# HandSomeWay/myGauHuman

Hardware: AMD Instinct MI355X
Metric: frames/sec fwd+bwd @1024^2, 200k Gaussians (higher is better)
Workload: dtype f32

## Files before the change

### mygauhuman_amd/csrc/geometry.hip

```cpp
#include "expand.h"
#include "gsr_common.h"
#include "project.h"
#include "sh_math.h"

namespace gsr {

constexpr int SH_M = 16;
constexpr int SH_ROW = SH_M * 3;
constexpr int SH_HALF = SH_ROW / 2;
constexpr int SH_LDS_ROW = 28;
constexpr int SH_CPT = SH_HALF / 4;

template <bool STAGE_SH>
__global__ __launch_bounds__(PRE_BLOCK) void preprocess_forward_kernel(const PreprocessArgs a) {
  __shared__ uint32_t wave_tot[PRE_BLOCK / WAVE];
  __shared__ __attribute__((aligned(16))) float s_sh[STAGE_SH ? PRE_BLOCK * SH_LDS_ROW : 4];
  const int i = blockIdx.x * PRE_BLOCK + threadIdx.x;
  float4 second[STAGE_SH ? SH_CPT : 1];
  if (STAGE_SH) {
    const int first = blockIdx.x * PRE_BLOCK;
    const int nrows = min(PRE_BLOCK, a.P - first);
    if (a.sh_half) {
      const uint4 *slab = reinterpret_cast<const uint4 *>(reinterpret_cast<const _Float16 *>(a.shs) + (size_t)first * SH_ROW);
#pragma unroll
// ... 67 lines not shown
            want_sh = true;
          } else {
            rgb = sh_to_rgb(a.D, p, a.campos, a.shs + (size_t)i * a.M * 3, clamp_bits);
          }
          my_radius = radi;
          tiles = area;
          rec.x = pix;
          rec.y = piy;
          rec.conic_a = cv.z * det_inv;
          rec.conic_b = -cv.y * det_inv;
          rec.conic_c = cv.x * det_inv;
          rec.opacity = a.opacities[i];
          rec.depth = pv.z;
          rec.r = rgb.x;
          rec.g = rgb.y;
          rec.b = rgb.z;
          const float o = rec.opacity, t255 = 255.0f * o;
          float hx = __builtin_inff(), hy = __builtin_inff();
          if (o == o) {
            if (!(t255 >= 1.0f)) {
              hx = hy = -1.0e30f;
            } else if (cv.x > 0.f && cv.z > 0.f && det > 0.f) {
              const float tau2 = 2.0f * (logf(t255) + 0.02f);
              hx = sqrtf(tau2 * cv.x) * 1.0001f + 0.01f;
              hy = sqrtf(tau2 * cv.z) * 1.0001f + 0.01f;
            }
          }
          rec.hx = hx;
          rec.hy = hy;
        }
      }
    }
  }
  if (STAGE_SH) {
    float3 d0;
    const ShDir dir = sh_dir(p, a.campos, d0);
    float res[3] = {0.f, 0.f, 0.f};
    __syncthreads();
    if (want_sh) sh_accumulate<0, SH_M / 2>(a.D, dir, &s_sh[threadIdx.x * SH_LDS_ROW], res);
    __syncthreads();
    {
      const int nrows = min(PRE_BLOCK, a.P - blockIdx.x * PRE_BLOCK);
      if (a.sh_half) {
#pragma unroll
        for (int j = 0; j < SH_CPT / 2; j++) {
          const int e = (int)threadIdx.x + j * PRE_BLOCK, row = e / (SH_CPT / 2), c8 = e % (SH_CPT / 2);
          if (row < nrows) {
            const _Float16 *hv = reinterpret_cast<const _Float16 *>(&second[j]);
            float *dst = &s_sh[row * SH_LDS_ROW + 8 * c8];
#pragma unroll
            for (int e2 = 0; e2 < 8; e2++) dst[e2] = (float)hv[e2];
          }
        }
      } else {
#pragma unroll
        for (int j = 0; j < SH_CPT; j++) {
          const int e = (int)threadIdx.x + j * PRE_BLOCK, row = e / SH_CPT, c4 = e % SH_CPT;
          if (row < nrows) *reinterpret_cast<float4 *>(&s_sh[row * SH_LDS_ROW + 4 * c4]) = second[j];
        }
      }
    }
    __syncthreads();
    if (want_sh) {
      sh_accumulate<SH_M / 2, SH_M>(a.D, dir, &s_sh[threadIdx.x * SH_LDS_ROW], res);
      const float3 rgb = sh_finish(res, clamp_bits);
      rec.r = rgb.x;
      rec.g = rgb.y;
      rec.b = rgb.z;
    }
  }
  if (i < a.P) {
    a.radii[i] = my_radius;
    a.geom.tiles_touched[i] = tiles;
    a.geom.clamped[i] = (uint8_t)clamp_bits;
    float4 *dst = reinterpret_cast<float4 *>(a.geom.recs + i);
    dst[0] = make_float4(rec.x, rec.y, rec.conic_a, rec.conic_b);
    dst[1] = make_float4(rec.conic_c, rec.opacity, rec.depth, rec.r);
    dst[2] = make_float4(rec.g, rec.b, rec.hx, rec.hy);
    if (a.zero_rows) {
      float4 *row = reinterpret_cast<float4 *>(a.geom.grad_rows + (size_t)i * GROWX);
#pragma unroll
      for (int k = 0; k < GROWX / 4; k++) row[k] = make_float4(0.f, 0.f, 0.f, 0.f);
    }
  }
  const uint32_t incl_w = wave_incl_scan(tiles);
  const int wave = threadIdx.x / WAVE, lane = threadIdx.x % WAVE;
  if (lane == WAVE - 1) wave_tot[wave] = incl_w;
  __syncthreads();
  uint32_t base = 0;
#pragma unroll
  for (int w = 0; w < PRE_BLOCK / WAVE; w++)
    if (w < wave) base += wave_tot[w];
  const uint32_t incl = base + incl_w;
  if (i < a.P) a.geom.block_incl[i] = incl;
  if (threadIdx.x == PRE_BLOCK - 1) a.geom.block_sums[blockIdx.x] = incl;
}

int launch_preprocess_forward(const PreprocessArgs &a, hipStream_t stream) {
  if (a.P <= 0) return GSR_OK;
  const bool stage = a.shs && !a.colors_precomp && a.M == SH_M && (reinterpret_cast<size_t>(a.shs) % 16 == 0);
  if (a.sh_half && a.shs && !a.colors_precomp && !stage) {
    set_error("fp16 SH storage needs 16 coefficients per Gaussian and a 16-byte aligned array");
    return GSR_EINVAL;
  }
  if (stage)
    hipLaunchKernelGGL(preprocess_forward_kernel<true>, dim3(pre_blocks(a.P)), dim3(PRE_BLOCK), 0, stream, a);
  else
    hipLaunchKernelGGL(preprocess_forward_kernel<false>, dim3(pre_blocks(a.P)), dim3(PRE_BLOCK), 0, stream, a);
  return GSR_OK;
}

__global__ void mark_visible_kernel(int P, const float *means3D, const float *view, uint8_t *present) {
  const int i = blockIdx.x * blockDim.x + threadIdx.x;
  if (i >= P) return;
  const float3 p = make_float3(means3D[3 * i], means3D[3 * i + 1], means3D[3 * i + 2]);
  const float z = view[2] * p.x + view[6] * p.y + view[10] * p.z + view[14];
// ... 104 lines not shown
```

### mygauhuman_amd/csrc/gsr_api.hip

```cpp
#include <stdarg.h>
#include <stdio.h>
#include <string.h>

#include <atomic>
#include <mutex>
#include <string>
#include <unordered_map>
#include <utility>
#include <vector>

#include "gsr_common.h"

namespace gsr {

static thread_local std::string g_error;

void set_error(const char *fmt, ...) {
  char buf[1024];
  va_list ap;
  va_start(ap, fmt);
  vsnprintf(buf, sizeof(buf), fmt, ap);
  va_end(ap);
  g_error = buf;
}
// ... 88 lines not shown
  } else if (!strcmp(key, "bucket_sort_merged")) {
    if (v != 0 && v != 1) return bad("0 or 1");
    o.bucket_sort_merged = v;
  } else if (!strcmp(key, "blend_sort")) {
    if (v != 0 && v != 1) return bad("0 or 1");
    o.blend_sort = v;
  } else if (!strcmp(key, "tile_order")) {
    if (v < 0 || v > 3) return bad("0 (natural order), 1 (longest lists first), 2 / 3 (2 x 2 / 4 x 2 tile blocks by summed length, a block per XCD)");
    o.tile_order = v;
  } else if (!strcmp(key, "tile_cull")) {
    if (v != 0 && v != 1) return bad("0 or 1");
    o.tile_cull = v;
  } else if (!strcmp(key, "blend_bwd_reduce")) {
    if (v < 0 || v > 4) return bad("0 (permlane / DPP folds), 3 (LDS folds: default); experiments: 1 (MFMA on folded rows), 2 (transposed MFMA contraction), 4 (LDS folds, the round-3 kernel)");
    if (experiment(v == 1 || v == 2 || v == 4)) return GSR_EINVAL;
    o.blend_bwd_reduce = v;
  } else if (!strcmp(key, "blend_layout")) {
    if (v != 0 && v != 1) return bad("0 (quadrant waves) or 1 (experiment: 4x4 blocks, four survivors per step)");
    if (experiment(v == 1)) return GSR_EINVAL;
    o.blend_layout = v;
  } else if (!strcmp(key, "blend_tail_cut")) {
    if (v < 0 || v > 16) return bad("0 .. 16 (sixteenths of the busy tiles at the end of the visiting order)");
    o.blend_tail_cut = v;
  } else if (!strcmp(key, "blend_segments")) {
    if (v < 0 || v > 64) return bad("0 (never) or the outlier threshold in quarters of the frame's mean list length (4 .. 64)");
    o.blend_segments = v;
  } else if (!strcmp(key, "blend_prio")) {
    if (v < 0 || v > 4) return bad("0, 1 (issue priority by list length); experiments: 2..4 (MEASUREMENT ONLY: render the longest lists alone)");
    if (experiment(v >= 2)) return GSR_EINVAL;
    o.blend_prio = v;
  } else if (!strcmp(key, "bake_batch_cells")) {
    if (v < 0 || v > 1000) return bad("0 (as many as the workspace holds) or 1 .. 1000");
    o.bake_batch_cells = v;
  } else if (!strcmp(key, "debug_no_atomics")) {
    if (v != 0 && v != 1) return bad("0 or 1");
    o.debug_no_atomics = v;
  } else if (!strcmp(key, "deterministic")) {
    if (v != 0 && v != 1) return bad("0 or 1");
    o.deterministic = v;
  } else {
    set_error("unknown tuning key %s", key);
    return GSR_EINVAL;
  }
  return GSR_OK;
}

static int readback_u32x2(const uint32_t *dev, uint32_t *out, hipStream_t stream) {
  ApiState &st = S();
  uint32_t *pinned = nullptr;
  {
    std::lock_guard<std::mutex> lock(st.pin_mutex);
    if (!st.pin_free.empty()) {
      pinned = st.pin_free.back();
      st.pin_free.pop_back();
    }
  }
  if (!pinned) GSR_HIP(hipHostMalloc(reinterpret_cast<void **>(&pinned), 64, hipHostMallocDefault));
  hipError_t e = hipMemcpyAsync(pinned, dev, 2 * sizeof(uint32_t), hipMemcpyDeviceToHost, stream);
  if (e == hipSuccess) e = hipStreamSynchronize(stream);
  out[0] = pinned[0];
  out[1] = pinned[1];
  {
    std::lock_guard<std::mutex> lock(st.pin_mutex);
    st.pin_free.push_back(pinned);
  }
  GSR_HIP(e);
// ... 200 lines not shown
}

int forward_stage_a(const FwdIn &in, const GeomState &geom, int *radii, hipStream_t stream, bool skip_scan = false) {
  const int grid_x = (in.width + TILE - 1) / TILE, grid_y = (in.height + TILE - 1) / TILE;
  PreprocessArgs pa;
  memset(&pa, 0, sizeof(pa));
  pa.P = in.P;
  pa.D = in.D;
  pa.M = in.M;
  pa.means3D = in.means3D;
  pa.scales = in.scales;
  pa.rotations = in.rotations;
  pa.opacities = in.opacities;
  pa.shs = in.shs;
  pa.cov3D_precomp = in.cov3D_precomp;
  pa.colors_precomp = in.colors_precomp;
  pa.scale_modifier = in.scale_modifier;
  pa.view = in.viewmatrix;
  pa.proj = in.projmatrix;
  pa.campos = in.cam_pos;
  pa.W = in.width;
  pa.H = in.height;
  pa.grid_x = grid_x;
  pa.grid_y = grid_y;
  pa.tan_fovx = in.tan_fovx;
  pa.tan_fovy = in.tan_fovy;
  pa.focal_y = in.height / (2.0f * in.tan_fovy);
  pa.focal_x = in.width / (2.0f * in.tan_fovx);
  pa.radii = radii;
  pa.geom = geom;
  pa.prefiltered = in.prefiltered;
  pa.sh_half = in.sh_half;
  pa.zero_rows = (in.debug & GSR_FWD_ZERO_ROWS) ? 1 : 0;
  if (in.prefiltered) GSR_HIP(zero_async(geom.total + 1, sizeof(uint32_t), stream));
  prof_begin(PROF_PREPROCESS_FWD, stream);
  int rc = launch_preprocess_forward(pa, stream);
  prof_end(PROF_PREPROCESS_FWD, stream);
  if (rc != GSR_OK) return rc;
  GSR_LAUNCH_CHECK(stream, in.debug & 1);
  if (skip_scan) return GSR_OK;
  prof_begin(PROF_SCAN, stream);
  rc = launch_scan_block_sums(geom, in.P, stream);
  prof_end(PROF_SCAN, stream);
  if (rc != GSR_OK) return rc;
  GSR_LAUNCH_CHECK(stream, in.debug & 1);
  return GSR_OK;
}

int forward_stage_b(const FwdIn &in, const GeomState &geom, BinningState &bin, const ImageState &img, const int *radii,
                    long R_host, size_t capacity, uint32_t *dev_status, hipStream_t stream, bool scan_fused = false) {
  const Options opt = options_for(stream);
  const int grid_x = (in.width + TILE - 1) / TILE, grid_y = (in.height + TILE - 1) / TILE;
  const size_t tiles = (size_t)grid_x * grid_y;
  int rc;
  const bool bucket = R_host < 0 || opt.binning_mode == GSR_BINNING_TILE_BUCKET;
  const bool fwd_sorts = bucket && forward_sorts_lists(opt, in.n_extra) && bucket_uses_hist(opt, in.P, tiles, capacity);
  prof_begin(PROF_BINNING, stream);
  if (bucket) {
    const int segments = (opt.tile_order == 1 && opt.blend_layout == 0 && !opt.blend_fwd_dma && (in.n_extra != 0 || opt.blend_fwd_waves == 4))
                             ? (opt.blend_segments | (opt.blend_tail_cut << 8)) : 0;
    rc = bucket_binning(geom, radii, in.P, grid_x, grid_y, capacity, R_host < 0, bin, img.ranges, img.order, img.ckpt_base, segments,
                        dev_status, in.prefiltered != 0, scan_fused, fwd_sorts, opt, stream, in.debug & 1);
    if (rc != GSR_OK) return rc;
  } else {
    const size_t R = (size_t)R_host;
    const int end_bit = 32 + (int)higher_msb((uint32_t)tiles);
// ... 327 lines not shown
  pb.means3D = means3D;
  pb.shs = shs;
  pb.scales = scales;
  pb.rotations = rotations;
  pb.cov3D = cov3D_precomp ? cov3D_precomp : geom.cov3D;
  pb.radii = radii;
  pb.clamped = geom.clamped;
  pb.scale_modifier = scale_modifier;
  pb.view = viewmatrix;
  pb.proj = projmatrix;
  pb.campos = campos;
  pb.W = width;
  pb.H = height;
  pb.tan_fovx = tan_fovx;
  pb.tan_fovy = tan_fovy;
  pb.focal_y = height / (2.0f * tan_fovy);
  pb.focal_x = width / (2.0f * tan_fovx);
  pb.grad_rows = geom.grad_rows;
  pb.grow = grow;
  pb.clear_rows = (flags & GSR_BWD_ROWS_ZEROED) ? 1 : 0;
  pb.CE = n_extra;
  pb.sh_half = sh_dtype == GSR_SH_F16 ? 1 : 0;
  pb.dL_dextra = dL_dextra;
  pb.recs = geom.recs;
  pb.dL_dmean2D = dL_dmean2D;
  pb.dL_dconic = dL_dconic;
  pb.dL_dopacity = dL_dopacity;
  pb.dL_dcolor = dL_dcolor;
  pb.dL_dmean3D = dL_dmean3D;
  pb.dL_dcov3D = dL_dcov3D;
  pb.dL_dsh = dL_dsh;
  pb.dL_dscale = dL_dscale;
  pb.dL_drot = dL_drot;
  prof_begin(PROF_PREPROCESS_BWD, stream);
  rc = launch_preprocess_backward(pb, stream);
  prof_end(PROF_PREPROCESS_BWD, stream);
  if (det_rows) {
    (void)hipStreamSynchronize(stream);
    (void)hipFree(det_rows);
  }
  if (rc != GSR_OK) return rc;
  GSR_LAUNCH_CHECK(stream, debug);
  return GSR_OK;
}

int gsr_rasterize_backward_ex(int P, int D, int M, int R, const float *background, int width, int height, const float *means3D,
                              const float *shs, const float *colors_precomp, const float *alphas, const float *scales,
                              float scale_modifier, const float *rotations, const float *cov3D_precomp, const float *viewmatrix,
                              const float *projmatrix, const float *campos, float tan_fovx, float tan_fovy, const int *radii,
                              char *geom_buffer, char *binning_buffer, char *image_buffer, const float *dL_dpix,
                              const float *dL_ddepths, const float *dL_dalphas, float *dL_dmean2D, float *dL_dconic,
                              float *dL_dopacity, float *dL_dcolor, float *dL_dmean3D, float *dL_dcov3D, float *dL_dsh,
                              float *dL_dscale, float *dL_drot, int debug, const float *extra_features, int n_extra,
                              const float *const *dL_dout_extra, float *dL_dextra, int sh_dtype, gsr_stream_t stream) {
  return rasterize_backward_impl(nullptr, nullptr, P, D, M, R, background, width, height, means3D, shs, colors_precomp, alphas, scales,
                                 scale_modifier, rotations, cov3D_precomp, viewmatrix, projmatrix, campos, tan_fovx, tan_fovy, radii,
                                 geom_buffer, binning_buffer, image_buffer, dL_dpix, dL_ddepths, dL_dalphas, dL_dmean2D, dL_dconic,
                                 dL_dopacity, dL_dcolor, dL_dmean3D, dL_dcov3D, dL_dsh, dL_dscale, dL_drot, debug, extra_features,
                                 n_extra, dL_dout_extra, dL_dextra, sh_dtype, stream);
}

int gsr_rasterize_backward_colors(int P, int R, int width, int height, char *geom_buffer, char *binning_buffer, char *image_buffer,
                                  const float *dL_dpix, float *dL_dcolor, int n_extra, const float *const *dL_dout_extra,
                                  float *dL_dextra, int debug, gsr_stream_t stream_) {
  hipStream_t stream = reinterpret_cast<hipStream_t>(stream_);
  if (P < 0 || R < 0 || width <= 0 || height <= 0) {
// ... 213 lines not shown
```

### mygauhuman_amd/csrc/gsr_common.h

```cpp
#pragma once
#include <hip/hip_runtime.h>
#include <stdint.h>
#include <stddef.h>

#include "../../include/gsr.h"

namespace gsr {

constexpr int TILE = 16;
constexpr int WAVE = 64;
constexpr int PRE_BLOCK = 256;

struct alignas(16) SplatRec {
  float x, y, conic_a, conic_b;
  float conic_c, opacity, depth, r;
  float g, b, hx, hy;
};
static_assert(sizeof(SplatRec) == 48, "SplatRec layout");

constexpr int GROW = 16;

constexpr int GROWX = 32;
constexpr int CE_MAX = 18;

struct GeomState {
  SplatRec *recs;
  float *cov3D;
  uint8_t *clamped;
  uint32_t *tiles_touched;
  uint32_t *point_offsets;
  int *internal_radii;
  uint32_t *block_incl;
  uint32_t *block_sums;
  uint32_t *block_prefix;
  uint32_t *total;
  float *grad_rows;
};
struct BinningState {
  uint64_t *keys_a;
  uint32_t *vals_a;
  uint64_t *keys_s;
  uint32_t *vals_s;
  uint32_t *hist;
  uint32_t *tile_counts;
  uint32_t *tile_cursor;
};
struct ImageState {
  float *final_T;
  uint32_t *n_contrib;
  uint2 *ranges;
  uint32_t *order;
  uint32_t *ckpt_base;
  float *ckpt;
};

inline size_t align_up(size_t v, size_t a) { return (v + a - 1) / a * a; }
template <typename T>
inline void carve(uintptr_t &p, T *&out, size_t count) {
  p = align_up(p, 256);
  out = reinterpret_cast<T *>(p);
  p += count * sizeof(T);
}
inline uintptr_t carve_begin(const void *chunk) { return reinterpret_cast<uintptr_t>(chunk); }

inline int pre_blocks(int P) { return (P + PRE_BLOCK - 1) / PRE_BLOCK; }
constexpr int SORT_ITEMS = 16;
constexpr int SORT_BLOCK = 256;
constexpr int SORT_TILE = SORT_ITEMS * SORT_BLOCK;
inline size_t sort_blocks(size_t n) { return (n + SORT_TILE - 1) / SORT_TILE; }
inline size_t sort_hist_words(size_t n) { return 256 * (sort_blocks(n) ? sort_blocks(n) : 1) + 256; }

inline GeomState geom_from_chunk(char *chunk_, size_t P, size_t *end = nullptr) {
  GeomState g;
  uintptr_t chunk = carve_begin(chunk_);
  size_t nb = (size_t)pre_blocks((int)P);
  carve(chunk, g.recs, P);
  carve(chunk, g.cov3D, P * 6);
  carve(chunk, g.clamped, P);
  carve(chunk, g.tiles_touched, P);
  carve(chunk, g.point_offsets, P);
  carve(chunk, g.internal_radii, P);
  carve(chunk, g.block_incl, P);
  carve(chunk, g.block_sums, nb);
  carve(chunk, g.block_prefix, nb);
  carve(chunk, g.total, 4);
  carve(chunk, g.grad_rows, P * GROWX);
  if (end) *end = chunk;
  return g;
}
inline size_t geom_bytes(size_t P) {
  size_t end = 0;
  geom_from_chunk(nullptr, P, &end);
  return end + 256;
}
inline BinningState binning_from_chunk(char *chunk_, size_t R, size_t tiles = 0, size_t *end = nullptr) {
  BinningState b;
  uintptr_t chunk = carve_begin(chunk_);
  size_t n = R ? R : 1;
  carve(chunk, b.keys_a, n);
  carve(chunk, b.vals_a, n);
  carve(chunk, b.keys_s, n);
  carve(chunk, b.vals_s, n);
  carve(chunk, b.hist, sort_hist_words(n));
  b.tile_counts = b.tile_cursor = nullptr;
  if (tiles) {
    carve(chunk, b.tile_counts, tiles * 16);
    carve(chunk, b.tile_cursor, tiles);
  }
  if (end) *end = chunk;
  return b;
}
inline size_t binning_bytes(size_t R, size_t tiles) {
  size_t end = 0;
  binning_from_chunk(nullptr, R, tiles ? tiles : 1, &end);
  return end + 256;
}
#if defined(__HIPCC__)
#define GSR_HD __host__ __device__
#else
// ... 52 lines not shown
  do {                                                                       \
    int _rc = ::gsr::check_hip((expr), #expr, __FILE__, __LINE__);           \
    if (_rc != GSR_OK) return _rc;                                           \
  } while (0)
#define GSR_LAUNCH_CHECK(stream, debug)                                      \
  do {                                                                       \
    GSR_HIP(hipGetLastError());                                              \
    if (debug) GSR_HIP(hipStreamSynchronize(stream));                        \
  } while (0)

enum ProfStage { PROF_PREPROCESS_FWD = 0, PROF_SCAN = 1, PROF_BINNING = 2, PROF_BLEND_FWD = 3, PROF_BLEND_BWD = 4,
                 PROF_PREPROCESS_BWD = 5, PROF_BLEND_BWD_COLORS = 6, PROF_NSTAGES = 7 };
void prof_begin(int stage, hipStream_t stream);
void prof_end(int stage, hipStream_t stream);

struct Options {
  int binning_mode = GSR_BINNING_TILE_BUCKET;
  int tile_cull = 1;
  int tile_order = 1;
  int bucket_hist = 1;
  int bucket_sort_merged = 1;
  int blend_sort = 1;
  int bucket_cstride = 4;
  int blend_fwd_dma = 0;
  int blend_fwd_waves = 4;
  int blend_bwd_waves = 4;
  int blend_bwd_reduce = 3;
  int deterministic = 0;
  int blend_layout = 0;
  int blend_tail_cut = 0;
  int blend_segments = 8;
  int blend_prio = 1;
  int bake_batch_cells = 0;
  int debug_no_atomics = 0;
};
Options options_for(hipStream_t stream);

struct PreprocessArgs {
  int P, D, M;
  const float *means3D, *scales, *rotations, *opacities, *shs, *cov3D_precomp, *colors_precomp;
  float scale_modifier;
  const float *view, *proj, *campos;
  int W, H, grid_x, grid_y;
  float tan_fovx, tan_fovy, focal_x, focal_y;
  int *radii;
  GeomState geom;
  int prefiltered;
  int sh_half;
  int zero_rows;
};
int launch_preprocess_forward(const PreprocessArgs &a, hipStream_t stream);
int launch_mark_visible(int P, const float *means3D, const float *view, uint8_t *present, hipStream_t stream);
int launch_scan_block_sums(const GeomState &g, int P, hipStream_t stream);
int launch_duplicate(const GeomState &g, const int *radii, int P, int grid_x, int grid_y, uint64_t *keys,
                     uint32_t *vals, hipStream_t stream);
int radix_sort_u64(size_t n, const uint64_t *in_k, const uint32_t *in_v, uint64_t *x_k, uint32_t *x_v, uint64_t *y_k,
                   uint32_t *y_v, int end_bit, uint32_t *hist, hipStream_t stream, int debug);
int radix_sort_u32(size_t n, const uint32_t *in_k, const uint32_t *in_v, uint32_t *x_k, uint32_t *x_v, uint32_t *y_k,
                   uint32_t *y_v, int end_bit, uint32_t *hist, hipStream_t stream, int debug);
inline int radix_passes(int end_bit) { return (end_bit + 7) / 8; }
int launch_tile_ranges(size_t R, const uint64_t *keys_sorted, uint2 *ranges, size_t tiles, hipStream_t stream);

struct BlendFwdArgs {
  const uint32_t *order;
  const uint2 *ranges;
  uint32_t *point_list;
  const SplatRec *recs;
  const uint64_t *unsorted;
  uint64_t *keys_sorted;
  int W, H, grid_x, grid_y;
  const float *bg;
  float *out_color, *out_depth, *out_alpha, *final_T;
  uint32_t *n_contrib;
  const float *extra;
  int CE;
  float *out_extra;
  int list_prio;
  const uint32_t *ckpt_base;
  float *ckpt;
  unsigned long long *trace;
};
int launch_blend_forward(const BlendFwdArgs &a, const Options &opt, hipStream_t stream);
// ... 59 lines not shown
struct BlendColorsBwdArgs {
  const uint32_t *order;
  const uint2 *ranges;
  const uint32_t *point_list;
  const SplatRec *recs;
  int W, H, grid_x, grid_y;
  const float *g_img[CB_IMAGES];
  int n_img;
  uint64_t col0;
  uint32_t col_mask;
  float *dL_dextra;
  float *dL_dcolor;
  int list_prio;
};
int launch_blend_colors_backward(const BlendColorsBwdArgs &a, hipStream_t stream);

struct PreprocessBwdArgs {
  int P, D, M;
  const float *means3D, *shs, *scales, *rotations, *cov3D;
  const int *radii;
  const uint8_t *clamped;
  float scale_modifier;
  const float *view, *proj, *campos;
  int W, H;
  float tan_fovx, tan_fovy, focal_x, focal_y;
  float *grad_rows;
  int grow;
  int clear_rows;
  int CE;
  float *dL_dextra;
  const SplatRec *recs;
  float *dL_dmean2D, *dL_dconic, *dL_dopacity, *dL_dcolor, *dL_dmean3D, *dL_dcov3D, *dL_dsh, *dL_dscale, *dL_drot;
  int sh_half;
};
int launch_preprocess_backward(const PreprocessBwdArgs &a, hipStream_t stream);

int launch_query_recs(int what, int P, const GeomState &g, void *dst, hipStream_t stream);

int bucket_binning(const GeomState &g, const int *radii, int P, int grid_x, int grid_y, size_t capacity, bool device_sized,
                   BinningState &b, uint2 *ranges, uint32_t *order, uint32_t *ckpt_base, int segments, uint32_t *dev_status,
                   bool check_prefilter, bool scan_fused, bool fwd_sorts, const Options &opt, hipStream_t stream, int debug);
bool bucket_uses_hist(const Options &opt, int P, size_t tiles, size_t capacity);
int bucket_sort_lists(const uint2 *ranges, uint64_t *bucket, uint32_t *point_list, uint64_t *keys_sorted, uint32_t *big_list,
                      uint32_t *big_count, size_t tiles, hipStream_t stream);

}

#if defined(__HIPCC__)
namespace gsr {

__device__ __forceinline__ int f2i_sat(float f) {
  if (f != f) return 0;
  if (f >= 2147483648.0f) return 2147483647;
  if (f <= -2147483648.0f) return (-2147483647 - 1);
  return (int)f;
}

__device__ __forceinline__ void tile_rect(float px, float py, int radius, int gx, int gy, int &x0, int &y0, int &x1,
                                          int &y1) {
  const float r = (float)radius;
  x0 = min(gx, max(0, f2i_sat((px - r) / (float)TILE)));
  y0 = min(gy, max(0, f2i_sat((py - r) / (float)TILE)));
  x1 = min(gx, max(0, f2i_sat((px + r + (float)(TILE - 1)) / (float)TILE)));
  y1 = min(gy, max(0, f2i_sat((py + r + (float)(TILE - 1)) / (float)TILE)));
}

// ... 74 lines not shown
```

### mygauhuman_amd/csrc/preprocess_bwd.hip

```cpp
#include "gsr_common.h"
#include "sh_math.h"

namespace gsr {

__device__ __forceinline__ void cov3d_backward(const float3 sc, float mod, const float4 q, const float *d, float *dL_dscale,
                                               float *dL_drot) {
  const float r = q.x, x = q.y, y = q.z, z = q.w;
  float R[3][3];
  R[0][0] = 1.f - 2.f * (y * y + z * z);
  R[0][1] = 2.f * (x * y - r * z);
  R[0][2] = 2.f * (x * z + r * y);
  R[1][0] = 2.f * (x * y + r * z);
  R[1][1] = 1.f - 2.f * (x * x + z * z);
  R[1][2] = 2.f * (y * z - r * x);
  R[2][0] = 2.f * (x * z - r * y);
  R[2][1] = 2.f * (y * z + r * x);
  R[2][2] = 1.f - 2.f * (x * x + y * y);
  const float s[3] = {mod * sc.x, mod * sc.y, mod * sc.z};
  float M[3][3];
#pragma unroll
  for (int c = 0; c < 3; c++)
#pragma unroll
    for (int rr = 0; rr < 3; rr++) M[c][rr] = s[rr] * R[c][rr];
  const float dS[3][3] = {{d[0], 0.5f * d[1], 0.5f * d[2]}, {0.5f * d[1], d[3], 0.5f * d[4]}, {0.5f * d[2], 0.5f * d[4], d[5]}};
// ... 198 lines not shown
#pragma unroll
    for (int k = 0; k < 4; k++) a.dL_drot[4 * (size_t)i + k] = dq[k];
  }
}

constexpr int BSH_M = 16, BSH_ROW = BSH_M * 3;
constexpr int BSH_HALF = BSH_ROW / 2;
constexpr int BSH_LDS_ROW = 28;
constexpr int BSH_CPT = BSH_HALF / 4;
constexpr int BWD_BLOCK = 128;

template <bool STAGE_SH>
__global__ __launch_bounds__(BWD_BLOCK) void preprocess_backward_kernel(const PreprocessBwdArgs a) {
  __shared__ __attribute__((aligned(16))) float s_sh[STAGE_SH ? BWD_BLOCK * BSH_LDS_ROW : 4];
  const int i = blockIdx.x * BWD_BLOCK + threadIdx.x;
  if (a.CE > 0) {
    const int first = blockIdx.x * BWD_BLOCK;
    const int nrows = min(BWD_BLOCK, a.P - first);
    const float *src = a.grad_rows + (size_t)first * a.grow + 9;
    float *dst = a.dL_dextra + (size_t)first * a.CE;
    for (int e = threadIdx.x; e < nrows * a.CE; e += BWD_BLOCK) {
      const int r = e / a.CE, c = e - r * a.CE;
      dst[e] = src[(size_t)r * a.grow + c];
    }
    if (a.clear_rows) {
      __syncthreads();
      float *rows = a.grad_rows + (size_t)first * a.grow;
      for (int e = threadIdx.x; e < nrows * (a.grow - 12); e += BWD_BLOCK) {
        const int r = e / (a.grow - 12), c = e - r * (a.grow - 12);
        rows[(size_t)r * a.grow + 12 + c] = 0.f;
      }
    }
  }
  if (STAGE_SH) {
    const int first = blockIdx.x * BWD_BLOCK;
    const int nrows = min(BWD_BLOCK, a.P - first);
    float4 second[BSH_CPT];
    if (a.sh_half) {
      const uint4 *slab = reinterpret_cast<const uint4 *>(reinterpret_cast<const _Float16 *>(a.shs) + (size_t)first * BSH_ROW);
#pragma unroll
      for (int j = 0; j < BSH_CPT / 2; j++) {
        const int e = (int)threadIdx.x + j * BWD_BLOCK, row = e / (BSH_CPT / 2), c8 = e % (BSH_CPT / 2);
        if (row < nrows) {
          const uint4 v = slab[row * (BSH_ROW / 8) + c8];
          second[j] = __builtin_bit_cast(float4, slab[row * (BSH_ROW / 8) + BSH_CPT / 2 + c8]);
          const _Float16 *hv = reinterpret_cast<const _Float16 *>(&v);
          float *dst = &s_sh[row * BSH_LDS_ROW + 8 * c8];
#pragma unroll
          for (int e2 = 0; e2 < 8; e2++) dst[e2] = (float)hv[e2];
        }
      }
    } else {
      const float4 *slab = reinterpret_cast<const float4 *>(a.shs + (size_t)first * BSH_ROW);
#pragma unroll
      for (int j = 0; j < BSH_CPT; j++) {
        const int e = (int)threadIdx.x + j * BWD_BLOCK, row = e / BSH_CPT, c4 = e % BSH_CPT;
        if (row < nrows) {
          *reinterpret_cast<float4 *>(&s_sh[row * BSH_LDS_ROW + 4 * c4]) = slab[row * (BSH_ROW / 4) + c4];
          second[j] = slab[row * (BSH_ROW / 4) + BSH_CPT + c4];
        }
      }
    }
    DeferredSh d;
    d.live = false;
    if (i < a.P) preprocess_backward_one<true>(a, i, nullptr, nullptr, &d);
    float3 d0 = make_float3(1.f, 0.f, 0.f);
    ShDir dir = {};
    float dd[9] = {0.f, 0.f, 0.f, 0.f, 0.f, 0.f, 0.f, 0.f, 0.f};
    if (d.live) dir = sh_dir(d.mean, a.campos, d0);
    float *mine = &s_sh[threadIdx.x * BSH_LDS_ROW];
    float4 *out = reinterpret_cast<float4 *>(a.dL_dsh + (size_t)first * BSH_ROW);
    __syncthreads();
    if (d.live) {
      sh_backward_range<0, BSH_M / 2>(a.D, dir, mine, d.dRGB, dd);
    } else if (i < a.P) {
#pragma unroll
      for (int k = 0; k < BSH_HALF; k++) mine[k] = 0.f;
    }
    __syncthreads();
#pragma unroll
    for (int j = 0; j < BSH_CPT; j++) {
      const int e = (int)threadIdx.x + j * BWD_BLOCK, row = e / BSH_CPT, c4 = e % BSH_CPT;
      if (row < nrows) {
        float4 *cell = reinterpret_cast<float4 *>(&s_sh[row * BSH_LDS_ROW + 4 * c4]);
        out[row * (BSH_ROW / 4) + c4] = *cell;
        if (!a.sh_half) *cell = second[j];
      }
    }
    if (a.sh_half) {
      __syncthreads();
#pragma unroll
      for (int j = 0; j < BSH_CPT / 2; j++) {
        const int e = (int)threadIdx.x + j * BWD_BLOCK, row = e / (BSH_CPT / 2), c8 = e % (BSH_CPT / 2);
        if (row < nrows) {
          const _Float16 *hv = reinterpret_cast<const _Float16 *>(&second[j]);
          float *dst = &s_sh[row * BSH_LDS_ROW + 8 * c8];
#pragma unroll
          for (int e2 = 0; e2 < 8; e2++) dst[e2] = (float)hv[e2];
        }
      }
    }
    __syncthreads();
// ... 40 lines not shown
```

### mygauhuman_amd/csrc/sh_math.h

```cpp
#pragma once
#include "gsr_common.h"

namespace gsr {

constexpr float kSH0 = 0.28209479177387814f;
constexpr float kSH1 = 0.4886025119029199f;
constexpr float kSH2[5] = {1.0925484305920792f, -1.0925484305920792f, 0.31539156525252005f, -1.0925484305920792f,
                           0.5462742152960396f};
constexpr float kSH3[7] = {-0.5900435899266435f, 2.890611442640554f, -0.4570457994644658f, 0.3731763325901154f,
                           -0.4570457994644658f, 1.445305721320277f,  -0.5900435899266435f};

__device__ __forceinline__ float3 sh_to_rgb(int deg, const float3 pos, const float *campos, const float *sh,
                                            uint32_t &clamp_bits) {
  const float dx0 = pos.x - campos[0], dy0 = pos.y - campos[1], dz0 = pos.z - campos[2];
  const float len = sqrtf(dx0 * dx0 + dy0 * dy0 + dz0 * dz0);
  const float x = dx0 / len, y = dy0 / len, z = dz0 / len;
  float out[3];
  clamp_bits = 0;
#pragma unroll
  for (int ch = 0; ch < 3; ch++) {
#define S(k) sh[(k) * 3 + ch]
    float res = kSH0 * S(0);
    if (deg > 0) {
      res = res - kSH1 * y * S(1) + kSH1 * z * S(2) - kSH1 * x * S(3);
// ... 107 lines not shown
  const float len = sqrtf(d0.x * d0.x + d0.y * d0.y + d0.z * d0.z);
  ShDir d;
  d.x = d0.x / len;
  d.y = d0.y / len;
  d.z = d0.z / len;
  d.xx = d.x * d.x;
  d.yy = d.y * d.y;
  d.zz = d.z * d.z;
  d.xy = d.x * d.y;
  d.yz = d.y * d.z;
  d.xz = d.x * d.z;
  return d;
}
template <int K>
__device__ __forceinline__ float sh_weight(const ShDir &d) {
  if constexpr (K == 0) return kSH0;
  if constexpr (K == 1) return -kSH1 * d.y;
  if constexpr (K == 2) return kSH1 * d.z;
  if constexpr (K == 3) return -kSH1 * d.x;
  if constexpr (K == 4) return kSH2[0] * d.xy;
  if constexpr (K == 5) return kSH2[1] * d.yz;
  if constexpr (K == 6) return kSH2[2] * (2.0f * d.zz - d.xx - d.yy);
  if constexpr (K == 7) return kSH2[3] * d.xz;
  if constexpr (K == 8) return kSH2[4] * (d.xx - d.yy);
  if constexpr (K == 9) return kSH3[0] * d.y * (3.0f * d.xx - d.yy);
  if constexpr (K == 10) return kSH3[1] * d.xy * d.z;
  if constexpr (K == 11) return kSH3[2] * d.y * (4.0f * d.zz - d.xx - d.yy);
  if constexpr (K == 12) return kSH3[3] * d.z * (2.0f * d.zz - 3.0f * d.xx - 3.0f * d.yy);
  if constexpr (K == 13) return kSH3[4] * d.x * (4.0f * d.zz - d.xx - d.yy);
  if constexpr (K == 14) return kSH3[5] * d.z * (d.xx - d.yy);
  if constexpr (K == 15) return kSH3[6] * d.x * (d.xx - 3.0f * d.yy);
  return 0.f;
}
template <int K>
__device__ __forceinline__ float3 sh_weight_grad(const ShDir &d) {
  if constexpr (K == 1) return make_float3(0.f, -kSH1, 0.f);
  if constexpr (K == 2) return make_float3(0.f, 0.f, kSH1);
  if constexpr (K == 3) return make_float3(-kSH1, 0.f, 0.f);
  if constexpr (K == 4) return make_float3(kSH2[0] * d.y, kSH2[0] * d.x, 0.f);
  if constexpr (K == 5) return make_float3(0.f, kSH2[1] * d.z, kSH2[1] * d.y);
  if constexpr (K == 6) return make_float3(kSH2[2] * 2.f * -d.x, kSH2[2] * 2.f * -d.y, kSH2[2] * 2.f * 2.f * d.z);
  if constexpr (K == 7) return make_float3(kSH2[3] * d.z, 0.f, kSH2[3] * d.x);
  if constexpr (K == 8) return make_float3(kSH2[4] * 2.f * d.x, kSH2[4] * 2.f * -d.y, 0.f);
  if constexpr (K == 9) return make_float3(kSH3[0] * 3.f * 2.f * d.xy, kSH3[0] * 3.f * (d.xx - d.yy), 0.f);
  if constexpr (K == 10) return make_float3(kSH3[1] * d.yz, kSH3[1] * d.xz, kSH3[1] * d.xy);
  if constexpr (K == 11)
    return make_float3(kSH3[2] * -2.f * d.xy, kSH3[2] * (-3.f * d.yy + 4.f * d.zz - d.xx), kSH3[2] * 4.f * 2.f * d.yz);
  if constexpr (K == 12)
    return make_float3(kSH3[3] * -3.f * 2.f * d.xz, kSH3[3] * -3.f * 2.f * d.yz, kSH3[3] * 3.f * (2.f * d.zz - d.xx - d.yy));
  if constexpr (K == 13)
    return make_float3(kSH3[4] * (-3.f * d.xx + 4.f * d.zz - d.yy), kSH3[4] * -2.f * d.xy, kSH3[4] * 4.f * 2.f * d.xz);
  if constexpr (K == 14) return make_float3(kSH3[5] * 2.f * d.xz, kSH3[5] * -2.f * d.yz, kSH3[5] * (d.xx - d.yy));
  if constexpr (K == 15) return make_float3(kSH3[6] * 3.f * (d.xx - d.yy), kSH3[6] * -3.f * 2.f * d.xy, 0.f);
  return make_float3(0.f, 0.f, 0.f);
}
constexpr int sh_band_of(int k) { return k == 0 ? 0 : k < 4 ? 1 : k < 9 ? 2 : 3; }

template <int LO, int HI, int K = LO>
__device__ __forceinline__ void sh_accumulate(int deg, const ShDir &d, const float *part, float (&res)[3]) {
  if constexpr (K < HI) {
    if (deg >= sh_band_of(K)) {
      const float w = sh_weight<K>(d);
#pragma unroll
      for (int ch = 0; ch < 3; ch++) {
        const float t = w * part[(K - LO) * 3 + ch];
        res[ch] = K == 0 ? t : res[ch] + t;
      }
    }
    sh_accumulate<LO, HI, K + 1>(deg, d, part, res);
  }
}
__device__ __forceinline__ float3 sh_finish(float (&res)[3], uint32_t &clamp_bits) {
  clamp_bits = 0;
#pragma unroll
  for (int ch = 0; ch < 3; ch++) {
    res[ch] += 0.5f;
    if (res[ch] < 0) clamp_bits |= 1u << ch;
    res[ch] = fmaxf(res[ch], 0.0f);
  }
  return make_float3(res[0], res[1], res[2]);
}

template <int LO, int HI, int K = LO>
__device__ __forceinline__ void sh_backward_range(int deg, const ShDir &d, float *part, const float (&dRGB)[3], float (&dd)[9]) {
  if constexpr (K < HI) {
    float *c = part + (K - LO) * 3;
    if (deg >= sh_band_of(K)) {
      const float w = sh_weight<K>(d);
      if constexpr (K > 0) {
        const float3 g = sh_weight_grad<K>(d);
#pragma unroll
        for (int ch = 0; ch < 3; ch++) {
          const float s = c[ch];
          dd[ch] += g.x * s;
          dd[3 + ch] += g.y * s;
          dd[6 + ch] += g.z * s;
        }
      }
#pragma unroll
      for (int ch = 0; ch < 3; ch++) c[ch] = w * dRGB[ch];
    } else {
      c[0] = c[1] = c[2] = 0.f;
    }
    sh_backward_range<LO, HI, K + 1>(deg, d, part, dRGB, dd);
  }
}
__device__ __forceinline__ void sh_backward_finish(const float3 d0, const float (&dRGB)[3], const float (&dd)[9], float *dL_dmean) {
  const float dd0 = dd[0] * dRGB[0] + dd[1] * dRGB[1] + dd[2] * dRGB[2];
  const float dd1 = dd[3] * dRGB[0] + dd[4] * dRGB[1] + dd[5] * dRGB[2];
  const float dd2 = dd[6] * dRGB[0] + dd[7] * dRGB[1] + dd[8] * dRGB[2];
  const float sum2 = d0.x * d0.x + d0.y * d0.y + d0.z * d0.z;
  const float inv32 = 1.0f / sqrtf(sum2 * sum2 * sum2);
  dL_dmean[0] += ((+sum2 - d0.x * d0.x) * dd0 - d0.y * d0.x * dd1 - d0.z * d0.x * dd2) * inv32;
  dL_dmean[1] += (-d0.x * d0.y * dd0 + (sum2 - d0.y * d0.y) * dd1 - d0.z * d0.y * dd2) * inv32;
  dL_dmean[2] += (-d0.x * d0.z * dd0 - d0.y * d0.z * dd1 + (sum2 - d0.z * d0.z) * dd2) * inv32;
}

__device__ __forceinline__ void sh_basis(int deg, float x, float y, float z, float *w) {
  w[0] = kSH0;
  if (deg > 0) {
    w[1] = -kSH1 * y;
    w[2] = kSH1 * z;
    w[3] = -kSH1 * x;
    if (deg > 1) {
      const float xx = x * x, yy = y * y, zz = z * z, xy = x * y, yz = y * z, xz = x * z;
      w[4] = kSH2[0] * xy;
      w[5] = kSH2[1] * yz;
      w[6] = kSH2[2] * (2.f * zz - xx - yy);
      w[7] = kSH2[3] * xz;
      w[8] = kSH2[4] * (xx - yy);
      if (deg > 2) {
        w[9] = kSH3[0] * y * (3.f * xx - yy);
        w[10] = kSH3[1] * xy * z;
        w[11] = kSH3[2] * y * (4.f * zz - xx - yy);
        w[12] = kSH3[3] * z * (2.f * zz - 3.f * xx - 3.f * yy);
        w[13] = kSH3[4] * x * (4.f * zz - xx - yy);
        w[14] = kSH3[5] * z * (xx - yy);
// ... 8 lines not shown
```

Baseline: 2767.

## Precompute SH direction Jacobian in forward preprocess and reuse it in backward

While the SH coefficients are already staged in LDS during the forward preprocess, the kernel now also computes the 3x9 direction Jacobian (dColor/ddir contracted per channel) and stores 9 floats per Gaussian. The backward preprocess then reads this Jacobian instead of reloading the SH coefficients, so it only writes dL_dsh and skips the coefficient read. A header word records the SH degree so the backward pass can check that the cache is valid. This trades 48 coefficient reads per Gaussian in backward for 9 extra writes in forward and 9 reads in backward, plus extra ALU work in forward. It also uses a fused-contract direction helper, which may change rounding slightly.

```diff
diff --git a/mygauhuman_amd/csrc/geometry.hip b/mygauhuman_amd/csrc/geometry.hip
--- a/mygauhuman_amd/csrc/geometry.hip
+++ b/mygauhuman_amd/csrc/geometry.hip
@@ -123,12 +123,20 @@
       }
     }
   }
+  const bool jac = STAGE_SH && a.sh_jac && a.D > 0;
+  ShDir dirj = {};
+  float dd[9] = {0.f, 0.f, 0.f, 0.f, 0.f, 0.f, 0.f, 0.f, 0.f};
   if (STAGE_SH) {
     float3 d0;
     const ShDir dir = sh_dir(p, a.campos, d0);
     float res[3] = {0.f, 0.f, 0.f};
-    __syncthreads();
-    if (want_sh) sh_accumulate<0, SH_M / 2>(a.D, dir, &s_sh[threadIdx.x * SH_LDS_ROW], res);
+    float3 d0j;
+    if (jac) dirj = sh_dir_fused(p, a.campos, d0j);
+    __syncthreads();
+    if (want_sh) {
+      sh_accumulate<0, SH_M / 2>(a.D, dir, &s_sh[threadIdx.x * SH_LDS_ROW], res);
+      if (jac) sh_jacobian_range<0, SH_M / 2>(a.D, dirj, &s_sh[threadIdx.x * SH_LDS_ROW], dd);
+    }
     __syncthreads();
     {
       const int nrows = min(PRE_BLOCK, a.P - blockIdx.x * PRE_BLOCK);
@@ -160,6 +168,7 @@
       rec.b = rgb.z;
     }
   }
+  if (blockIdx.x == 0 && threadIdx.x == 0) a.geom.total[SH_JAC_HDR] = (STAGE_SH && a.sh_jac) ? sh_jac_word(a.D) : 0u;
   if (i < a.P) {
     a.radii[i] = my_radius;
     a.geom.tiles_touched[i] = tiles;
@@ -173,6 +182,12 @@
 #pragma unroll
       for (int k = 0; k < GROWX / 4; k++) row[k] = make_float4(0.f, 0.f, 0.f, 0.f);
     }
+  }
+  if (want_sh && jac) {
+    sh_jacobian_range<SH_M / 2, SH_M>(a.D, dirj, &s_sh[threadIdx.x * SH_LDS_ROW], dd);
+    float *dst = a.geom.sh_jac + 9 * (size_t)i;
+#pragma unroll
+    for (int k = 0; k < 9; k++) dst[k] = dd[k];
   }
   const uint32_t incl_w = wave_incl_scan(tiles);
   const int wave = threadIdx.x / WAVE, lane = threadIdx.x % WAVE;
diff --git a/mygauhuman_amd/csrc/gsr_api.hip b/mygauhuman_amd/csrc/gsr_api.hip
--- a/mygauhuman_amd/csrc/gsr_api.hip
+++ b/mygauhuman_amd/csrc/gsr_api.hip
@@ -144,6 +144,9 @@
   } else if (!strcmp(key, "bake_batch_cells")) {
     if (v < 0 || v > 1000) return bad("0 (as many as the workspace holds) or 1 .. 1000");
     o.bake_batch_cells = v;
+  } else if (!strcmp(key, "sh_jacobian")) {
+    if (v != 0 && v != 1) return bad("0 or 1");
+    o.sh_jacobian = v;
   } else if (!strcmp(key, "debug_no_atomics")) {
     if (v != 0 && v != 1) return bad("0 or 1");
     o.debug_no_atomics = v;
@@ -410,6 +413,7 @@
   pa.prefiltered = in.prefiltered;
   pa.sh_half = in.sh_half;
   pa.zero_rows = (in.debug & GSR_FWD_ZERO_ROWS) ? 1 : 0;
+  pa.sh_jac = (options_for(stream).sh_jacobian && in.n_extra == 0) ? 1 : 0;
   if (in.prefiltered) GSR_HIP(zero_async(geom.total + 1, sizeof(uint32_t), stream));
   prof_begin(PROF_PREPROCESS_FWD, stream);
   int rc = launch_preprocess_forward(pa, stream);
@@ -803,6 +807,10 @@
   pb.dL_dsh = dL_dsh;
   pb.dL_dscale = dL_dscale;
   pb.dL_drot = dL_drot;
+  if (opt.sh_jacobian && n_extra == 0 && !p1) {
+    pb.sh_jac = geom.sh_jac;
+    pb.sh_jac_hdr = geom.total + SH_JAC_HDR;
+  }
   prof_begin(PROF_PREPROCESS_BWD, stream);
   rc = launch_preprocess_backward(pb, stream);
   prof_end(PROF_PREPROCESS_BWD, stream);
diff --git a/mygauhuman_amd/csrc/gsr_common.h b/mygauhuman_amd/csrc/gsr_common.h
--- a/mygauhuman_amd/csrc/gsr_common.h
+++ b/mygauhuman_amd/csrc/gsr_common.h
@@ -35,6 +35,7 @@
   uint32_t *block_prefix;
   uint32_t *total;
   float *grad_rows;
+  float *sh_jac;
 };
 struct BinningState {
   uint64_t *keys_a;
@@ -69,6 +70,9 @@
 constexpr int SORT_TILE = SORT_ITEMS * SORT_BLOCK;
 inline size_t sort_blocks(size_t n) { return (n + SORT_TILE - 1) / SORT_TILE; }
 inline size_t sort_hist_words(size_t n) { return 256 * (sort_blocks(n) ? sort_blocks(n) : 1) + 256; }
+
+constexpr int SH_JAC_HDR = 3;
+constexpr uint32_t sh_jac_word(int D) { return (uint32_t)D + 1u; }
 
 inline GeomState geom_from_chunk(char *chunk_, size_t P, size_t *end = nullptr) {
   GeomState g;
@@ -85,6 +89,7 @@
   carve(chunk, g.block_prefix, nb);
   carve(chunk, g.total, 4);
   carve(chunk, g.grad_rows, P * GROWX);
+  carve(chunk, g.sh_jac, P * 9);
   if (end) *end = chunk;
   return g;
 }
@@ -203,6 +208,7 @@
   int blend_segments = 8;
   int blend_prio = 1;
   int bake_batch_cells = 0;
+  int sh_jacobian = 1;
   int debug_no_atomics = 0;
 };
 Options options_for(hipStream_t stream);
@@ -219,6 +225,7 @@
   int prefiltered;
   int sh_half;
   int zero_rows;
+  int sh_jac;
 };
 int launch_preprocess_forward(const PreprocessArgs &a, hipStream_t stream);
 int launch_mark_visible(int P, const float *means3D, const float *view, uint8_t *present, hipStream_t stream);
@@ -344,6 +351,8 @@
   const SplatRec *recs;
   float *dL_dmean2D, *dL_dconic, *dL_dopacity, *dL_dcolor, *dL_dmean3D, *dL_dcov3D, *dL_dsh, *dL_dscale, *dL_drot;
   int sh_half;
+  const float *sh_jac;
+  const uint32_t *sh_jac_hdr;
 };
 int launch_preprocess_backward(const PreprocessBwdArgs &a, hipStream_t stream);
 
diff --git a/mygauhuman_amd/csrc/preprocess_bwd.hip b/mygauhuman_amd/csrc/preprocess_bwd.hip
--- a/mygauhuman_amd/csrc/preprocess_bwd.hip
+++ b/mygauhuman_amd/csrc/preprocess_bwd.hip
@@ -254,7 +254,54 @@
       }
     }
   }
-  if (STAGE_SH) {
+  if (STAGE_SH && a.sh_jac && a.sh_jac_hdr[0] == sh_jac_word(a.D)) {
+    const int first = blockIdx.x * BWD_BLOCK;
+    const int nrows = min(BWD_BLOCK, a.P - first);
+    DeferredSh d;
+    d.live = false;
+    if (i < a.P) preprocess_backward_one<true>(a, i, nullptr, nullptr, &d);
+    float3 d0 = make_float3(1.f, 0.f, 0.f);
+    ShDir dir = {};
+    float dd[9] = {0.f, 0.f, 0.f, 0.f, 0.f, 0.f, 0.f, 0.f, 0.f};
+    if (d.live) {
+      dir = sh_dir_fused(d.mean, a.campos, d0);
+      if (a.D > 0) {
+#pragma unroll
+        for (int k = 0; k < 9; k++) dd[k] = a.sh_jac[9 * (size_t)i + k];
+      }
+    }
+    float *mine = &s_sh[threadIdx.x * BSH_LDS_ROW];
+    float4 *out = reinterpret_cast<float4 *>(a.dL_dsh + (size_t)first * BSH_ROW);
+    if (d.live) {
+      sh_gradient_range<0, BSH_M / 2>(a.D, dir, mine, d.dRGB);
+    } else if (i < a.P) {
+#pragma unroll
+      for (int k = 0; k < BSH_HALF; k++) mine[k] = 0.f;
+    }
+    __syncthreads();
+#pragma unroll
+    for (int j = 0; j < BSH_CPT; j++) {
+      const int e = (int)threadIdx.x + j * BWD_BLOCK, row = e / BSH_CPT, c4 = e % BSH_CPT;
+      if (row < nrows) out[row * (BSH_ROW / 4) + c4] = *reinterpret_cast<const float4 *>(&s_sh[row * BSH_LDS_ROW + 4 * c4]);
+    }
+    __syncthreads();
+    if (d.live) {
+      sh_gradient_range<BSH_M / 2, BSH_M>(a.D, dir, mine, d.dRGB);
+      sh_backward_finish(d0, d.dRGB, dd, d.dm);
+      a.dL_dmean3D[3 * (size_t)i + 0] = d.dm[0];
+      a.dL_dmean3D[3 * (size_t)i + 1] = d.dm[1];
+      a.dL_dmean3D[3 * (size_t)i + 2] = d.dm[2];
+    } else if (i < a.P) {
+#pragma unroll
+      for (int k = 0; k < BSH_HALF; k++) mine[k] = 0.f;
+    }
+    __syncthreads();
+#pragma unroll
+    for (int j = 0; j < BSH_CPT; j++) {
+      const int e = (int)threadIdx.x + j * BWD_BLOCK, row = e / BSH_CPT, c4 = e % BSH_CPT;
+      if (row < nrows) out[row * (BSH_ROW / 4) + BSH_CPT + c4] = *reinterpret_cast<const float4 *>(&s_sh[row * BSH_LDS_ROW + 4 * c4]);
+    }
+  } else if (STAGE_SH) {
     const int first = blockIdx.x * BWD_BLOCK;
     const int nrows = min(BWD_BLOCK, a.P - first);
     float4 second[BSH_CPT];
@@ -289,7 +336,7 @@
     float3 d0 = make_float3(1.f, 0.f, 0.f);
     ShDir dir = {};
     float dd[9] = {0.f, 0.f, 0.f, 0.f, 0.f, 0.f, 0.f, 0.f, 0.f};
-    if (d.live) dir = sh_dir(d.mean, a.campos, d0);
+    if (d.live) dir = sh_dir_fused(d.mean, a.campos, d0);
     float *mine = &s_sh[threadIdx.x * BSH_LDS_ROW];
     float4 *out = reinterpret_cast<float4 *>(a.dL_dsh + (size_t)first * BSH_ROW);
     __syncthreads();
diff --git a/mygauhuman_amd/csrc/sh_math.h b/mygauhuman_amd/csrc/sh_math.h
--- a/mygauhuman_amd/csrc/sh_math.h
+++ b/mygauhuman_amd/csrc/sh_math.h
@@ -163,8 +163,25 @@
   if constexpr (K == 15) return kSH3[6] * d.x * (d.xx - 3.0f * d.yy);
   return 0.f;
 }
+__device__ __forceinline__ ShDir sh_dir_fused(const float3 pos, const float *campos, float3 &d0) {
+#pragma clang fp contract(fast)
+  d0 = make_float3(pos.x - campos[0], pos.y - campos[1], pos.z - campos[2]);
+  const float len = sqrtf(d0.x * d0.x + d0.y * d0.y + d0.z * d0.z);
+  ShDir d;
+  d.x = d0.x / len;
+  d.y = d0.y / len;
+  d.z = d0.z / len;
+  d.xx = d.x * d.x;
+  d.yy = d.y * d.y;
+  d.zz = d.z * d.z;
+  d.xy = d.x * d.y;
+  d.yz = d.y * d.z;
+  d.xz = d.x * d.z;
+  return d;
+}
 template <int K>
 __device__ __forceinline__ float3 sh_weight_grad(const ShDir &d) {
+#pragma clang fp contract(fast)
   if constexpr (K == 1) return make_float3(0.f, -kSH1, 0.f);
   if constexpr (K == 2) return make_float3(0.f, 0.f, kSH1);
   if constexpr (K == 3) return make_float3(-kSH1, 0.f, 0.f);
@@ -212,28 +229,54 @@
   return make_float3(res[0], res[1], res[2]);
 }
 
+template <int K>
+__device__ __forceinline__ void sh_jacobian_term(const ShDir &d, const float *c, float (&dd)[9]) {
+#pragma clang fp contract(fast)
+  if constexpr (K > 0) {
+    const float3 g = sh_weight_grad<K>(d);
+#pragma unroll
+    for (int ch = 0; ch < 3; ch++) {
+      const float s = c[ch];
+      dd[ch] += g.x * s;
+      dd[3 + ch] += g.y * s;
+      dd[6 + ch] += g.z * s;
+    }
+  }
+}
 template <int LO, int HI, int K = LO>
 __device__ __forceinline__ void sh_backward_range(int deg, const ShDir &d, float *part, const float (&dRGB)[3], float (&dd)[9]) {
   if constexpr (K < HI) {
     float *c = part + (K - LO) * 3;
     if (deg >= sh_band_of(K)) {
       const float w = sh_weight<K>(d);
-      if constexpr (K > 0) {
-        const float3 g = sh_weight_grad<K>(d);
-#pragma unroll
-        for (int ch = 0; ch < 3; ch++) {
-          const float s = c[ch];
-          dd[ch] += g.x * s;
-          dd[3 + ch] += g.y * s;
-          dd[6 + ch] += g.z * s;
-        }
-      }
+      sh_jacobian_term<K>(d, c, dd);
 #pragma unroll
       for (int ch = 0; ch < 3; ch++) c[ch] = w * dRGB[ch];
     } else {
       c[0] = c[1] = c[2] = 0.f;
     }
     sh_backward_range<LO, HI, K + 1>(deg, d, part, dRGB, dd);
+  }
+}
+template <int LO, int HI, int K = LO>
+__device__ __forceinline__ void sh_jacobian_range(int deg, const ShDir &d, const float *part, float (&dd)[9]) {
+  if constexpr (K < HI) {
+    if (deg >= sh_band_of(K)) sh_jacobian_term<K>(d, part + (K - LO) * 3, dd);
+    sh_jacobian_range<LO, HI, K + 1>(deg, d, part, dd);
+  }
+}
+template <int LO, int HI, int K = LO>
+__device__ __forceinline__ void sh_gradient_range(int deg, const ShDir &d, float *part, const float (&dRGB)[3]) {
+  if constexpr (K < HI) {
+    float *c = part + (K - LO) * 3;
+    if (deg >= sh_band_of(K)) {
+      const float w = sh_weight<K>(d);
+#pragma unroll
+      for (int ch = 0; ch < 3; ch++) c[ch] = w * dRGB[ch];
+    } else {
+      c[0] = c[1] = c[2] = 0.f;
+    }
+    sh_gradient_range<LO, HI, K + 1>(deg, d, part, dRGB);
   }
 }
 __device__ __forceinline__ void sh_backward_finish(const float3 d0, const float (&dRGB)[3], const float (&dd)[9], float *dL_dmean) {
```

New measurement: 2765. Within noise of the previous version (-0.1%).
